# microsoft/UniSpeech

Hardware: AMD Instinct MI355X
Metric: audio-seconds/sec pretraining, WavLM-Base 15s@16kHz (higher is better)
Workload: dtype bf16; 1 GPU; WavLM-Base (12L, d=768) pretrain fwd+bwd+grad-reduce+fused-Adam, bf16, batch=32x15s per GPU, masked-pred loss (BASELINE.json configs[1]); global_batch=32, frames_per_utt=749, parallelism=dp1, optimizer=fused Adam, fp32 master, clip 10

## Files before the change

include/wavlm_hip.h:

```cpp
#ifndef WAVLM_HIP_H
#define WAVLM_HIP_H
#include <stddef.h>
#include <stdint.h>
#ifdef __cplusplus
extern "C" {
#endif

#define WAVLM_HIP_ABI_VERSION 29
int wavlm_abi_version(void);

typedef struct wavlm_gemm_desc {
  int32_t dtype;
  int32_t c_dtype;
  int32_t M, N, K, KB;
  int32_t transA, transB;
  int64_t lda, ldb, ldc;
  int64_t sA_kb, sB_kb;
  int32_t batch_o, batch_i;
  int64_t sA_o, sA_i, sB_o, sB_i, sC_o, sC_i;
  const void* A;
  const void* B;
  void* C;
  float alpha;
  int32_t epi;
  const void* bias; int32_t bias_dtype; int64_t sBias_o, sBias_i;
  void* aux; int32_t aux_dtype; int64_t ld_aux, sAux_o, sAux_i;
  const void* res; int32_t res_dtype; int64_t ld_res, sRes_o, sRes_i;
  int32_t accumulate;
  int32_t split_k;
  void* workspace; uint64_t ws_bytes;
  void* colsum; int32_t colsum_dtype; int32_t colsum_accumulate;
} wavlm_gemm_desc;

uint64_t wavlm_gemm_workspace_bytes(const wavlm_gemm_desc* d);
int wavlm_gemm(const wavlm_gemm_desc* d, void* stream);
int wavlm_gemm_grouped(const wavlm_gemm_desc* d, int32_t n, void* stream);

int32_t wavlm_grid_blocks(void);
int32_t wavlm_split_single(int32_t M, int32_t N, int64_t ktiles, int32_t grid);
int32_t wavlm_split_grouped(int64_t tiles, int64_t ktiles, int32_t grid, int32_t forced);
int32_t wavlm_slabs_grouped(int64_t tiles, int64_t ktiles, int32_t grid, int32_t forced, int32_t balanced);
// ... 3 lines not shown
  const void* dy;
  const void* x;
  void* dW;
  int32_t N, K;
} wavlm_wgrad_item;
uint64_t wavlm_linear_wgrads_workspace_bytes(const wavlm_wgrad_item* items, int32_t n_items, int64_t rows);
int wavlm_linear_wgrads(const wavlm_wgrad_item* items, int32_t n_items, int64_t rows, int32_t c_dtype, void* workspace,
                        uint64_t ws_bytes, void* stream);


int wavlm_layernorm_fwd(const void* x, const void* r, void* y, void* s, float* mean, float* rstd, const void* gamma,
                        const void* beta, int64_t rows, int32_t D, float eps, int32_t dtype, int32_t param_dtype,
                        int32_t act, float p_in, uint64_t seed_in, float p_out, uint64_t seed_out, void* stream);
uint64_t wavlm_layernorm_bwd_workspace_bytes(int32_t D);
int wavlm_layernorm_bwd(const void* dy, const void* s, const float* mean, const float* rstd, const void* gamma,
                        const void* beta, void* dx, void* dr, const void* dx_add, void* dgamma, void* dbeta,
                        void* dr_colsum, int64_t rows, int32_t D, int32_t dtype, int32_t param_dtype, int32_t act,
                        float p_in, uint64_t seed_in, float p_out, uint64_t seed_out, float grad_scale,
                        int32_t accumulate_params, int32_t dr_incl_add, void* workspace, uint64_t ws_bytes, void* stream);
int wavlm_layernorm_bwd_seg(const void* dy, const void* s, const float* mean, const float* rstd, const void* gamma,
                            const void* beta, void* dx, void* dr, const void* dx_add, void* dgamma, void* dbeta,
                            void* dr_colsum, int64_t rows, int32_t D, int32_t dtype, int32_t param_dtype, int32_t act,
                            float p_in, uint64_t seed_in, float p_out, uint64_t seed_out, float grad_scale,
                            int32_t accumulate_params, int32_t dr_incl_add, int32_t dx_seg_rows, int32_t dx_seg_gap,
                            void* workspace, uint64_t ws_bytes, void* stream);

uint64_t wavlm_colsum_workspace_bytes(int32_t N);
int wavlm_colsum(const void* x, int64_t rows, int32_t N, int64_t ld, int32_t dtype, const uint8_t* include_mask,
                 const uint8_t* exclude_mask, void* out, int32_t out_dtype, int32_t accumulate, void* workspace,
                 uint64_t ws_bytes, void* stream);

int wavlm_select_rows(const void* x, void* y, const uint8_t* sel, const void* emb, const uint8_t* zero, int64_t rows,
                      int32_t D, int32_t dtype, int32_t emb_dtype, void* stream);
int wavlm_gather_rows(const void* src, const int32_t* idx, void* dst, int64_t n_out, int32_t D, int32_t dtype,
                      void* stream);
#define WL_CONV_RELAYOUT_MAX 8
typedef struct {
  const void* W[WL_CONV_RELAYOUT_MAX];
  void* Wf[WL_CONV_RELAYOUT_MAX];
  void* Wb[WL_CONV_RELAYOUT_MAX];
  int32_t Cout[WL_CONV_RELAYOUT_MAX], Cin[WL_CONV_RELAYOUT_MAX], k[WL_CONV_RELAYOUT_MAX], s[WL_CONV_RELAYOUT_MAX];
  int32_t n_layers, dtype;
} wavlm_conv_relayout_desc;
int wavlm_conv_weights_relayout(const wavlm_conv_relayout_desc* d, void* stream);
int wavlm_conv_wgrad_scatter(const wavlm_conv_relayout_desc* d, int32_t accumulate, void* stream);
int wavlm_axpby(const void* x, int32_t x_dtype, void* y, int32_t y_dtype, int64_t n, float a, float b, void* stream);
int wavlm_scale_dev(void* y, int32_t dtype, int64_t n, const float* scalar, float extra, void* stream);
int wavlm_dropout(const void* x, void* y, int64_t n, float p, uint64_t seed, int32_t dtype, void* stream);
int wavlm_dropout_add(const void* x, const void* r, void* y, int64_t n, float p, uint64_t seed, int32_t dtype, void* stream);
uint64_t wavlm_sumsq_workspace_bytes(void);
int wavlm_sumsq(const void* x, int32_t dtype, int64_t n, float scale, float* out, void* workspace, uint64_t ws_bytes,
                void* stream);

uint64_t wavlm_conv0_gn_workspace_bytes(int32_t B, int64_t T, int32_t C, int32_t stride);
int wavlm_conv0_gn_gelu_fwd(const void* wav, int32_t wav_dtype, const void* W, const void* gamma, const void* beta,
                            int32_t param_dtype, void* out, int32_t out_dtype, float* stats, int32_t B, int64_t T,
                            int32_t C, int32_t kw, int32_t stride, float eps, void* workspace, uint64_t ws_bytes,
                            void* stream);
uint64_t wavlm_conv0_gn_bwd_workspace_bytes(int32_t B, int64_t T, int32_t C, int32_t stride);
int wavlm_conv0_gn_gelu_bwd(const void* wav, int32_t wav_dtype, const void* W, const void* gamma, const void* beta,
                            int32_t param_dtype, const void* g, int32_t g_dtype, const float* stats, void* dW,
                            void* dgamma, void* dbeta, int32_t B, int64_t T, int32_t C, int32_t kw, int32_t stride,
                            float gscale, void* workspace, uint64_t ws_bytes, void* stream);

uint64_t wavlm_conv0_ln_fwd_workspace_bytes(void);
int wavlm_conv0_ln_gelu_fwd(const void* wav, int32_t wav_dtype, const void* W, const void* conv_bias, const void* gamma,
// ... 224 lines not shown
```

unispeech_amd/_lib.py:

```python
import ctypes as C
import os

_HERE = os.path.dirname(os.path.abspath(__file__))
LIB_PATH = os.environ.get("WAVLM_HIP_LIB") or os.path.join(_HERE, "lib", "libwavlm_hip.so")

_lib = None
ABI_VERSION = 29

F32, BF16, I16 = 0, 1, 2

c_i32, c_i64, c_u64, c_f32, c_vp = C.c_int32, C.c_int64, C.c_uint64, C.c_float, C.c_void_p


class ConvRelayoutDesc(C.Structure):
    _fields_ = [("W", c_vp * 8), ("Wf", c_vp * 8), ("Wb", c_vp * 8),
                ("Cout", c_i32 * 8), ("Cin", c_i32 * 8), ("k", c_i32 * 8), ("s", c_i32 * 8),
                ("n_layers", c_i32), ("dtype", c_i32)]


class GemmDesc(C.Structure):
    _fields_ = [
        ("dtype", c_i32), ("c_dtype", c_i32),
        ("M", c_i32), ("N", c_i32), ("K", c_i32), ("KB", c_i32),
        ("transA", c_i32), ("transB", c_i32),
        ("lda", c_i64), ("ldb", c_i64), ("ldc", c_i64),
        ("sA_kb", c_i64), ("sB_kb", c_i64),
        ("batch_o", c_i32), ("batch_i", c_i32),
        ("sA_o", c_i64), ("sA_i", c_i64), ("sB_o", c_i64), ("sB_i", c_i64), ("sC_o", c_i64), ("sC_i", c_i64),
        ("A", c_vp), ("B", c_vp), ("C", c_vp),
        ("alpha", c_f32), ("epi", c_i32),
        ("bias", c_vp), ("bias_dtype", c_i32), ("sBias_o", c_i64), ("sBias_i", c_i64),
        ("aux", c_vp), ("aux_dtype", c_i32), ("ld_aux", c_i64), ("sAux_o", c_i64), ("sAux_i", c_i64),
        ("res", c_vp), ("res_dtype", c_i32), ("ld_res", c_i64), ("sRes_o", c_i64), ("sRes_i", c_i64),
        ("accumulate", c_i32), ("split_k", c_i32),
        ("workspace", c_vp), ("ws_bytes", c_u64),
        ("colsum", c_vp), ("colsum_dtype", c_i32), ("colsum_accumulate", c_i32),
    ]


class WgradItem(C.Structure):
# ... 17 lines not shown
        ("tab", c_vp), ("kpm", c_vp),
        ("x", c_vp), ("r_in", c_vp), ("y", c_vp), ("r_out", c_vp),
        ("saved", c_vp), ("saved_bytes", c_u64), ("workspace", c_vp), ("ws_bytes", c_u64),
        ("dy", c_vp), ("dr_out", c_vp), ("dx", c_vp), ("dr_in", c_vp), ("dtab", c_vp),
    ]


GRAD_LISTENER = C.CFUNCTYPE(None, c_vp, c_u64, c_vp, c_vp)


SIGNATURES = {
    "wavlm_abi_version": (c_i32, []),
    "wavlm_gemm_workspace_bytes": (c_u64, [C.POINTER(GemmDesc)]),
    "wavlm_gemm": (c_i32, [C.POINTER(GemmDesc), c_vp]),
    "wavlm_gemm_grouped": (c_i32, [C.POINTER(GemmDesc), c_i32, c_vp]),
    "wavlm_grid_blocks": (c_i32, []),
    "wavlm_split_single": (c_i32, [c_i32, c_i32, c_i64, c_i32]),
    "wavlm_split_grouped": (c_i32, [c_i64, c_i64, c_i32, c_i32]),
    "wavlm_slabs_grouped": (c_i32, [c_i64, c_i64, c_i32, c_i32, c_i32]),
    "wavlm_wgrad_grouping": (c_i32, []),
    "wavlm_linear_wgrads_workspace_bytes": (c_u64, [C.POINTER(WgradItem), c_i32, c_i64]),
    "wavlm_linear_wgrads": (c_i32, [C.POINTER(WgradItem), c_i32, c_i64, c_i32, c_vp, c_u64, c_vp]),
    "wavlm_layernorm_fwd": (c_i32, [c_vp, c_vp, c_vp, c_vp, c_vp, c_vp, c_vp, c_vp, c_i64, c_i32, c_f32, c_i32, c_i32,
                                    c_i32, c_f32, c_u64, c_f32, c_u64, c_vp]),
    "wavlm_layernorm_bwd_workspace_bytes": (c_u64, [c_i32]),
    "wavlm_layernorm_bwd": (c_i32, [c_vp, c_vp, c_vp, c_vp, c_vp, c_vp, c_vp, c_vp, c_vp, c_vp, c_vp, c_vp, c_i64, c_i32, c_i32,
                                    c_i32, c_i32, c_f32, c_u64, c_f32, c_u64, c_f32, c_i32, c_i32, c_vp, c_u64, c_vp]),
    "wavlm_layernorm_bwd_seg": (c_i32, [c_vp, c_vp, c_vp, c_vp, c_vp, c_vp, c_vp, c_vp, c_vp, c_vp, c_vp, c_vp, c_i64, c_i32, c_i32,
                                        c_i32, c_i32, c_f32, c_u64, c_f32, c_u64, c_f32, c_i32, c_i32, c_i32, c_i32, c_vp, c_u64,
                                        c_vp]),
    "wavlm_colsum_workspace_bytes": (c_u64, [c_i32]),
    "wavlm_colsum": (c_i32, [c_vp, c_i64, c_i32, c_i64, c_i32, c_vp, c_vp, c_vp, c_i32, c_i32, c_vp, c_u64, c_vp]),
    "wavlm_select_rows": (c_i32, [c_vp, c_vp, c_vp, c_vp, c_vp, c_i64, c_i32, c_i32, c_i32, c_vp]),
    "wavlm_gather_rows": (c_i32, [c_vp, c_vp, c_vp, c_i64, c_i32, c_i32, c_vp]),
    "wavlm_conv_weights_relayout": (c_i32, [C.POINTER(ConvRelayoutDesc), c_vp]),
    "wavlm_conv_wgrad_scatter": (c_i32, [C.POINTER(ConvRelayoutDesc), c_i32, c_vp]),
    "wavlm_axpby": (c_i32, [c_vp, c_i32, c_vp, c_i32, c_i64, c_f32, c_f32, c_vp]),
    "wavlm_scale_dev": (c_i32, [c_vp, c_i32, c_i64, c_vp, c_f32, c_vp]),
    "wavlm_dropout": (c_i32, [c_vp, c_vp, c_i64, c_f32, c_u64, c_i32, c_vp]),
    "wavlm_dropout_add": (c_i32, [c_vp, c_vp, c_vp, c_i64, c_f32, c_u64, c_i32, c_vp]),
    "wavlm_sumsq_workspace_bytes": (c_u64, []),
    "wavlm_sumsq": (c_i32, [c_vp, c_i32, c_i64, c_f32, c_vp, c_vp, c_u64, c_vp]),
    "wavlm_conv0_gn_workspace_bytes": (c_u64, [c_i32, c_i64, c_i32, c_i32]),
    "wavlm_conv0_gn_gelu_fwd": (c_i32, [c_vp, c_i32, c_vp, c_vp, c_vp, c_i32, c_vp, c_i32, c_vp, c_i32, c_i64, c_i32,
                                        c_i32, c_i32, c_f32, c_vp, c_u64, c_vp]),
    "wavlm_conv0_gn_bwd_workspace_bytes": (c_u64, [c_i32, c_i64, c_i32, c_i32]),
    "wavlm_conv0_gn_gelu_bwd": (c_i32, [c_vp, c_i32, c_vp, c_vp, c_vp, c_i32, c_vp, c_i32, c_vp, c_vp, c_vp, c_vp,
                                        c_i32, c_i64, c_i32, c_i32, c_i32, c_f32, c_vp, c_u64, c_vp]),
    "wavlm_conv0_ln_fwd_workspace_bytes": (c_u64, []),
    "wavlm_conv0_ln_gelu_fwd": (c_i32, [c_vp, c_i32, c_vp, c_vp, c_vp, c_vp, c_i32, c_vp, c_i32, c_i32, c_i64, c_i32, c_i32,
                                        c_i32, c_f32, c_vp, c_u64, c_vp]),
    "wavlm_conv0_ln_bwd_workspace_bytes": (c_u64, [c_i32, c_i64, c_i32, c_i32]),
    "wavlm_conv0_ln_gelu_bwd": (c_i32, [c_vp, c_i32, c_vp, c_vp, c_vp, c_vp, c_i32, c_vp, c_i32, c_vp, c_vp, c_vp, c_vp, c_i32,
                                        c_i64, c_i32, c_i32, c_i32, c_f32, c_f32, c_vp, c_u64, c_vp]),
    "wavlm_relpos_gather": (c_i32, [c_vp, c_i32, c_vp, c_vp, c_i32, c_i32, c_vp]),
    "wavlm_relpos_scatter": (c_i32, [c_vp, c_vp, c_vp, c_i32, c_i32, c_i32, c_i32, c_vp]),
    "wavlm_gate_fwd": (c_i32, [c_vp, c_vp, c_vp, c_vp, c_vp, c_vp, c_vp, c_i32, c_i32, c_i32, c_i32, c_i32, c_i32,
                               c_vp]),
    "wavlm_gate_bwd_workspace_bytes": (c_u64, [c_i32, c_i32]),
    "wavlm_gate_bwd": (c_i32, [c_vp, c_vp, c_vp, c_vp, c_vp, c_vp, c_vp, c_vp, c_vp, c_vp, c_i32, c_i32, c_i32, c_i32,
                               c_i32, c_i32, c_i32, c_vp, c_u64, c_vp]),
    "wavlm_attn_softmax_fwd": (c_i32, [c_vp, c_vp, c_vp, c_vp, c_vp, c_vp, c_i32, c_i32, c_i32, c_i64, c_i64, c_i32,
                                       c_i32, c_f32, c_u64, c_vp]),
    "wavlm_attn_softmax_bwd_workspace_bytes": (c_u64, [c_i32, c_i32, c_i32]),
    "wavlm_attn_softmax_bwd": (c_i32, [c_vp, c_vp, c_vp, c_vp, c_vp, c_vp, c_vp, c_vp, c_vp, c_i32, c_i32, c_i32,
                                       c_i32, c_i64, c_i64, c_i32, c_i32, c_f32, c_u64, c_vp, c_u64, c_vp]),
# ... 127 lines not shown
```

unispeech_amd/csrc/rowops.hip:

```cpp
#include "common.hpp"
#include <stdlib.h>
#include "../../include/wavlm_hip.h"

__device__ __forceinline__ void load8(const float* p, float (&v)[8]) {
  const float4 a = *reinterpret_cast<const float4*>(p);
  const float4 b = *reinterpret_cast<const float4*>(p + 4);
  v[0] = a.x; v[1] = a.y; v[2] = a.z; v[3] = a.w; v[4] = b.x; v[5] = b.y; v[6] = b.z; v[7] = b.w;
}
__device__ __forceinline__ void load8(const bf16_t* p, float (&v)[8]) {
  const uint4 a = *reinterpret_cast<const uint4*>(p);
  v[0] = __uint_as_float(a.x << 16); v[1] = __uint_as_float(a.x & 0xffff0000u);
  v[2] = __uint_as_float(a.y << 16); v[3] = __uint_as_float(a.y & 0xffff0000u);
  v[4] = __uint_as_float(a.z << 16); v[5] = __uint_as_float(a.z & 0xffff0000u);
  v[6] = __uint_as_float(a.w << 16); v[7] = __uint_as_float(a.w & 0xffff0000u);
}
__device__ __forceinline__ void store8(float* p, const float (&v)[8]) {
  *reinterpret_cast<float4*>(p) = make_float4(v[0], v[1], v[2], v[3]);
  *reinterpret_cast<float4*>(p + 4) = make_float4(v[4], v[5], v[6], v[7]);
}
__device__ __forceinline__ void store8(bf16_t* p, const float (&v)[8]) {
  uint4 o;
  o.x = pack_bf16x2(v[0], v[1]); o.y = pack_bf16x2(v[2], v[3]);
  o.z = pack_bf16x2(v[4], v[5]); o.w = pack_bf16x2(v[6], v[7]);
  *reinterpret_cast<uint4*>(p) = o;
// ... 610 lines not shown
#pragma unroll
    for (int e = 0; e < 8; ++e) acc[c][e] = 0.f;
  for (long row = (long)blockIdx.x * 4 + wave; row < rows; row += (long)gridDim.x * 4) {
    if (inc && !inc[row]) continue;
    if (exc && exc[row]) continue;
#pragma unroll
    for (int c = 0; c < CS_MAXC; ++c) {
      const int ch = lane + 64 * c;
      if (ch < nch) {
        float v[8];
        load8(x + row * ld + ch * 8, v);
#pragma unroll
        for (int e = 0; e < 8; ++e) acc[c][e] += v[e];
      }
    }
  }
  float* pg = part + (long)blockIdx.x * N;
#pragma unroll
  for (int c = 0; c < CS_MAXC; ++c) {
    __syncthreads();
#pragma unroll
    for (int e = 0; e < 8; ++e) red[wave][lane * 8 + e] = acc[c][e];
    __syncthreads();
    for (int i = threadIdx.x; i < 512; i += 256) {
      const int ch = (i >> 3) + 64 * c;
      if (ch < nch) pg[ch * 8 + (i & 7)] = red[0][i] + red[1][i] + red[2][i] + red[3][i];
    }
  }
}

template <typename T, typename TP>
__global__ __launch_bounds__(256) void select_rows_kernel(const T* __restrict__ x, T* __restrict__ y,
    const unsigned char* __restrict__ sel, const TP* __restrict__ emb, const unsigned char* __restrict__ zero,
    long rows, int D) {
  const int nch = D >> 3;
  const long total = rows * nch;
  for (long i = (long)blockIdx.x * blockDim.x + threadIdx.x; i < total; i += (long)gridDim.x * blockDim.x) {
    const long row = i / nch; const int ch = (int)(i - row * nch);
    float v[8];
    if (zero && zero[row]) {
#pragma unroll
      for (int e = 0; e < 8; ++e) v[e] = 0.f;
    } else if (sel && sel[row]) {
      if (emb) load8(emb + ch * 8, v);
      else {
#pragma unroll
        for (int e = 0; e < 8; ++e) v[e] = 0.f;
      }
    } else {
      load8(x + row * D + ch * 8, v);
    }
    store8(y + row * D + ch * 8, v);
  }
}

template <typename T>
__global__ __launch_bounds__(256) void gather_rows_kernel(const T* __restrict__ src, const int* __restrict__ idx,
                                                           T* __restrict__ dst, long n_out, int D) {
  const int nch = D >> 3;
  const long total = n_out * nch;
  for (long i = (long)blockIdx.x * blockDim.x + threadIdx.x; i < total; i += (long)gridDim.x * blockDim.x) {
    const long row = i / nch; const int ch = (int)(i - row * nch);
    const int srow = idx[row];
    float v[8];
    if (srow >= 0) load8(src + (long)srow * D + ch * 8, v);
    else {
#pragma unroll
      for (int e = 0; e < 8; ++e) v[e] = 0.f;
    }
    store8(dst + row * D + ch * 8, v);
  }
}

__global__ __launch_bounds__(256) void axpby_kernel(const void* x, int xdt, void* y, int ydt, long n, float a, float b) {
  for (long i = (long)blockIdx.x * blockDim.x + threadIdx.x; i < n; i += (long)gridDim.x * blockDim.x) {
    float v = a * ld_elem(x, i, xdt);
    if (b != 0.f) v += b * ld_elem(y, i, ydt);
    st_elem(y, i, ydt, v);
  }
}


__global__ __launch_bounds__(256) void scale_dev_kernel(void* y, int ydt, long n, const float* __restrict__ s, float extra) {
// ... 288 lines not shown
  WL_LAUNCH(colsum_finish_kernel, dim3((unsigned)((n + 15) / 16)), dim3(1024), 0, st, part, nblk, (long)n, n, out, out_dtype,
            accumulate, 0L, (void*)nullptr, (void*)nullptr);
  return wl_check_launch();
}
extern "C" {

uint64_t wavlm_colsum_workspace_bytes(int32_t N) { return (uint64_t)CS_BLOCKS * N * sizeof(float); }

int wavlm_colsum(const void* x, int64_t rows, int32_t N, int64_t ld, int32_t dtype, const uint8_t* include_mask,
                 const uint8_t* exclude_mask, void* out, int32_t out_dtype, int32_t accumulate, void* workspace,
                 uint64_t ws_bytes, void* stream) {
  if (!x || !out || !workspace || rows < 0 || N <= 0 || (N & 7) || N > CS_MAXC * 512 || (ld & 7)) return WL_EINVAL;
  if (ws_bytes < wavlm_colsum_workspace_bytes(N)) return WL_EINVAL;
  hipStream_t st = (hipStream_t)stream;
  const unsigned grid = grid_for(rows > 0 ? rows : 1, 4, CS_BLOCKS);
  float* part = (float*)workspace;
  if (dtype == WL_F32)
    WL_LAUNCH((colsum_partial_kernel<float>), dim3(grid), dim3(256), 0, st, (const float*)x, (long)rows, (int)N,
                       (long)ld, include_mask, exclude_mask, part);
  else if (dtype == WL_BF16)
    WL_LAUNCH((colsum_partial_kernel<bf16_t>), dim3(grid), dim3(256), 0, st, (const bf16_t*)x, (long)rows, (int)N,
                       (long)ld, include_mask, exclude_mask, part);
  else return WL_EINVAL;
  int rc = wl_check_launch();
  if (rc != WL_OK) return rc;
  if (wl_fin_add(part, (int)grid, (long)N, N, out, out_dtype, accumulate)) return WL_OK;
  WL_LAUNCH(colsum_finish_kernel, dim3((unsigned)((N + 15) / 16)), dim3(1024), 0, st, part, (int)grid, (long)N,
                     (int)N, out, (int)out_dtype, (int)accumulate, 0L, (void*)nullptr, (void*)nullptr);
  rc = wl_check_launch();
  if (rc == WL_OK && accumulate) wl_notify_grad(out, (uint64_t)N * wl_esize(out_dtype), stream);
  return rc;
}

int wavlm_select_rows(const void* x, void* y, const uint8_t* sel, const void* emb, const uint8_t* zero, int64_t rows,
                      int32_t D, int32_t dtype, int32_t emb_dtype, void* stream) {
  if (!x || !y || rows < 0 || D <= 0 || (D & 7)) return WL_EINVAL;
  if (rows == 0) return WL_OK;
  hipStream_t st = (hipStream_t)stream;
  const unsigned grid = grid_for(rows * (D >> 3), 256, 4096);
#define SEL(T, TP) WL_LAUNCH((select_rows_kernel<T, TP>), dim3(grid), dim3(256), 0, st, (const T*)x, (T*)y, sel, \
    (const TP*)emb, zero, (long)rows, (int)D)
  if (dtype == WL_F32 && emb_dtype == WL_F32) SEL(float, float);
  else if (dtype == WL_BF16 && emb_dtype == WL_BF16) SEL(bf16_t, bf16_t);
  else if (dtype == WL_BF16 && emb_dtype == WL_F32) SEL(bf16_t, float);
  else return WL_EINVAL;
#undef SEL
  return wl_check_launch();
}

int wavlm_gather_rows(const void* src, const int32_t* idx, void* dst, int64_t n_out, int32_t D, int32_t dtype,
                      void* stream) {
  if (!src || !idx || !dst || n_out < 0 || D <= 0 || (D & 7)) return WL_EINVAL;
  if (n_out == 0) return WL_OK;
  hipStream_t st = (hipStream_t)stream;
  const unsigned grid = grid_for(n_out * (D >> 3), 256, 4096);
  if (dtype == WL_F32)
    WL_LAUNCH((gather_rows_kernel<float>), dim3(grid), dim3(256), 0, st, (const float*)src, idx, (float*)dst,
                       (long)n_out, (int)D);
  else if (dtype == WL_BF16)
    WL_LAUNCH((gather_rows_kernel<bf16_t>), dim3(grid), dim3(256), 0, st, (const bf16_t*)src, idx, (bf16_t*)dst,
                       (long)n_out, (int)D);
  else return WL_EINVAL;
  return wl_check_launch();
}

int wavlm_conv_weights_relayout(const wavlm_conv_relayout_desc* d, void* stream) {
  if (!d || d->n_layers < 1 || d->n_layers > WL_CONV_RELAYOUT_MAX || (d->dtype != WL_F32 && d->dtype != WL_BF16)) return WL_EINVAL;
  long mx = 0;
  for (int l = 0; l < d->n_layers; ++l) {
    if (!d->W[l] || !d->Wf[l] || d->Cout[l] <= 0 || d->Cin[l] <= 0 || d->k[l] <= 0 || d->s[l] <= 0 || d->s[l] > d->k[l]) return WL_EINVAL;
    const long n = (long)d->Cout[l] * d->Cin[l] * d->k[l];
    if (n > mx) mx = n;
  }
  const unsigned gx = grid_for(mx, 256, 8192);
  WL_LAUNCH(conv_weights_relayout_kernel, dim3(gx, (unsigned)d->n_layers), dim3(256), 0, (hipStream_t)stream, *d);
  return wl_check_launch();
}

int wavlm_conv_wgrad_scatter(const wavlm_conv_relayout_desc* d, int32_t accumulate, void* stream) {
  if (!d || d->n_layers < 1 || d->n_layers > WL_CONV_RELAYOUT_MAX || (d->dtype != WL_F32 && d->dtype != WL_BF16)) return WL_EINVAL;
// ... 82 lines not shown
```

unispeech_amd/functional.py:

```python
import os
import threading
import weakref

import torch

from . import ops

_SEED_CTR = [0]
USE_FUSED_ATTENTION = True
_ASP = os.environ.get("WAVLM_ATTN_STORE_P", "0")
ATTN_STORE_P = True if _ASP == "1" else ("bits" if _ASP in ("bits", "2") else False)


def next_seed():
    _SEED_CTR[0] += 1
    return (torch.initial_seed() * 0x9E3779B97F4A7C15 + _SEED_CTR[0] * 0xD1B54A32D192ED03) & 0xFFFFFFFFFFFFFFFF


def _rup(x, m):
    return (x + m - 1) // m * m


CHAIN_CONSUMERS = os.environ.get("WAVLM_CHAIN_CONSUMERS", "1") == "1"
WGRAD_GROUPING = None
SINK_LISTENERS = []


def h2d(a, dev):
    t = torch.from_numpy(a) if not torch.is_tensor(a) else a
    dev = torch.device(dev)
    if dev.type != "cuda" or t.device.type != "cpu" or t.numel() == 0:
        return t.to(dev)
    return t.pin_memory().to(dev, non_blocking=True)


_SINK_USES = {}


def reset_sink_uses():
    _SINK_USES.clear()
    _PADDED_GRAD[0] = None


def _sink_use(p, explicit=None):
    if not SINK_LISTENERS:
        return
    t = explicit if explicit is not None else _sink(p)
    if t is not None:
        k = t.data_ptr()
        _SINK_USES[k] = _SINK_USES.get(k, 0) + 1


def _sink_written(t):
    if not SINK_LISTENERS:
        return
    k = t.data_ptr()
    left = _SINK_USES.get(k, 1) - 1
    if left > 0:
        _SINK_USES[k] = left
        return
    _SINK_USES.pop(k, None)
    for cb in SINK_LISTENERS:
        cb(t)


def _sink(p):
# ... 716 lines not shown
            dqkv, dgate, dtab = ops.attn_fused_bwd(qkvc, O, dO.contiguous(), lse, gate, tab, kpm, H, scale, p_drop, seed,
                                                   dbias=sb.view(-1) if sb is not None else None, dbias_accumulate=True,
                                                   pstore=pstore)
            if sb is not None:
                _sink_written(sb)
            return dqkv, dgate, dtab, None, None, None, None, None, None, None
        qkvc, S, P, lse, gate, tab, kpm = ctx.saved_tensors
        B, T, D, H, hd, ld, scale, p_drop, seed = ctx.cfg
        D3 = 3 * D
        dev = dO.device
        dOc = dO.contiguous()
        dP = torch.empty((B * H, T, ld), dtype=P.dtype, device=dev)
        ops.gemm(dOc, qkvc, dP, T, T, hd, lda=D, ldb=D3, ldc=ld, batch=(B, H), sA=(T * D, hd), sB=(T * D3, hd),
                 b_off=2 * D, sC=(H * T * ld, T * ld))
        dS = torch.empty_like(dP)
        dgate = dtab = None
        if tab is not None:
            dgate = torch.empty((B, H, T), dtype=torch.float32, device=dev)
            dtab = torch.empty_like(tab)
        ops.attn_softmax_bwd(S, dP, lse, gate, tab, kpm, dS, dgate, dtab, B, H, T, ld, ld, p_drop, seed)
        dqkv = torch.empty_like(qkvc)
        ops.gemm(dS, qkvc, dqkv, T, hd, T, lda=ld, ldb=D3, ldc=D3, transB=True, batch=(B, H),
                 sA=(H * T * ld, T * ld), sB=(T * D3, hd), b_off=D, sC=(T * D3, hd), c_off=0, alpha=scale)
        ops.gemm(dS, qkvc, dqkv, T, hd, T, lda=ld, ldb=D3, ldc=D3, transA=True, transB=True, batch=(B, H),
                 sA=(H * T * ld, T * ld), sB=(T * D3, hd), b_off=0, sC=(T * D3, hd), c_off=D, alpha=scale)
        ops.gemm(P, dOc, dqkv, T, hd, T, lda=ld, ldb=D, ldc=D3, transA=True, transB=True, batch=(B, H),
                 sA=(H * T * ld, T * ld), sB=(T * D, hd), sC=(T * D3, hd), c_off=2 * D)
        return dqkv, dgate, dtab, None, None, None, None, None, None, None


class SelectRowsFn(torch.autograd.Function):

    @staticmethod
    def forward(ctx, x, sel, emb, zero):
        xc = x.contiguous()
        y = ops.select_rows(xc, sel, emb, zero)
        ctx.save_for_backward(sel, zero, emb)
        return y

    @staticmethod
    def backward(ctx, dy):
        sel, zero, emb = ctx.saved_tensors
        dyc = dy.contiguous()
        dx = ops.select_rows(dyc, sel, None, zero) if ctx.needs_input_grad[0] else None
        demb = None
        if emb is not None and sel is not None and ctx.needs_input_grad[2]:
            demb = ops.colsum(dyc.view(-1, dyc.shape[-1]), emb.dtype, include=sel, exclude=zero)
        return dx, None, demb, None


class GatherRowsFn(torch.autograd.Function):

    @staticmethod
    def forward(ctx, x2d, idx, inv_idx):
        ctx.save_for_backward(inv_idx)
        ctx.n = x2d.shape[0]
        if idx.numel() == 0:
            return x2d.new_empty((0, x2d.shape[1]))
        return ops.gather_rows(x2d.contiguous(), idx, idx.numel())

    @staticmethod
    def backward(ctx, dy):
        (inv_idx,) = ctx.saved_tensors
        if dy.shape[0] == 0:
            return dy.new_zeros((ctx.n, dy.shape[1])), None, None
        return ops.gather_rows(dy.contiguous(), inv_idx, ctx.n), None, None


class DropoutFn(torch.autograd.Function):
    @staticmethod
    def forward(ctx, x, p, seed):
        ctx.p, ctx.seed = p, seed
        return ops.dropout(x.contiguous(), p, seed)

    @staticmethod
    def backward(ctx, dy):
        return ops.dropout(dy.contiguous(), ctx.p, ctx.seed), None, None


def dropout(x, p, training=True):
    if not training or p <= 0:
# ... 245 lines not shown
```

unispeech_amd/ops.py:

```python
import ctypes as C
import os

import torch

from . import _lib
from ._lib import BF16, F32, ConvRelayoutDesc, GemmDesc, check

_WS = {}


def dt(t):
    if t.dtype == torch.float32:
        return F32
    if t.dtype == torch.bfloat16:
        return BF16
    raise TypeError("unsupported dtype %s (float32 / bfloat16 only)" % t.dtype)


def _dev(t):
    if not t.is_cuda:
        raise _lib.WavlmHipError("unispeech_amd kernels need a HIP device tensor (no CPU fallback)")
    return t.device


# ... 191 lines not shown
        if torch.is_tensor(dr_colsum):
            raise ValueError("dr_colsum sink needs dgamma / dbeta sinks")
        dr_colsum = torch.empty_like(gamma) if not acc else torch.zeros_like(gamma)
    L = _lib.lib()
    need = L.wavlm_layernorm_bwd_workspace_bytes(D)
    ws = workspace(dev, need)
    check(L.wavlm_layernorm_bwd_seg(ptr(dy), ptr(s), ptr(mean), ptr(rstd), ptr(gamma), ptr(beta), ptr(dx), ptr(dr),
                                    ptr(dx_add), ptr(dgamma), ptr(dbeta), ptr(dr_colsum), rows, D, dt(dy), dt(gamma), int(act),
                                    float(p_in), int(seed_in), float(p_out), int(seed_out), float(grad_scale), int(acc),
                                    int(bool(dr_incl_add)), seg_rows, seg_gap, ptr(ws), need, stream()), "wavlm_layernorm_bwd_seg")
    if padded is not None:
        dx._padded = padded
    return dx, dr, dgamma, dbeta, dr_colsum


def colsum(x2d, out_dtype, *, include=None, exclude=None, rows=None, N=None, ld=None, out=None, accumulate=False):
    dev = _dev(x2d)
    if rows is None:
        N = x2d.shape[-1]
        rows = x2d.numel() // N
        ld = N
        _contig(x2d)
    if out is None:
        out = torch.empty(N, dtype=out_dtype, device=dev)
        accumulate = False
    L = _lib.lib()
    need = L.wavlm_colsum_workspace_bytes(N)
    ws = workspace(dev, need)
    check(L.wavlm_colsum(ptr(x2d), rows, N, ld, dt(x2d), ptr(include), ptr(exclude), ptr(out), dt(out),
                         int(bool(accumulate)), ptr(ws), need, stream()), "wavlm_colsum")
    return out


def select_rows(x, sel, emb, zero):
    _dev(x); _contig(x)
    D = x.shape[-1]
    rows = x.numel() // D
    y = torch.empty_like(x)
    check(_lib.lib().wavlm_select_rows(ptr(x), ptr(y), ptr(sel), ptr(emb), ptr(zero), rows, D, dt(x),
                                       dt(emb) if emb is not None else dt(x), stream()), "wavlm_select_rows")
    return y


def gather_rows(src2d, idx, n_out):
    dev = _dev(src2d); _contig(src2d)
    D = src2d.shape[-1]
    dst = torch.empty((n_out, D), dtype=src2d.dtype, device=dev)
    check(_lib.lib().wavlm_gather_rows(ptr(src2d), ptr(idx), ptr(dst), n_out, D, dt(src2d), stream()),
          "wavlm_gather_rows")
    return dst


def _conv_desc(weights, specs):
    d = ConvRelayoutDesc()
    if len(weights) > 8:
        raise ValueError("at most 8 convolution layers per call")
    d.n_layers, d.dtype = len(weights), dt(weights[0])
    for l, (W, (k, s_)) in enumerate(zip(weights, specs)):
        _dev(W); _contig(W)
        Cout, Cin, kk = W.shape
        if kk != k:
            raise ValueError("kernel width of layer %d does not match its spec" % l)
        d.Cout[l], d.Cin[l], d.k[l], d.s[l] = Cout, Cin, k, s_
        d.W[l] = W.data_ptr()
    return d


def conv_weights_relayout(weights, specs, want_bwd):
    d = _conv_desc(weights, specs)
    Wf, Wb = [], []
    for l, (W, (k, s_)) in enumerate(zip(weights, specs)):
        Cout, Cin, _ = W.shape
        f = torch.empty((Cout, k * Cin), dtype=W.dtype, device=W.device)
# ... 544 lines not shown
```

unispeech_amd/pretrain.py:

```python
import math
from dataclasses import dataclass, field
from typing import Dict, List, Optional, Tuple

import numpy as np
import torch
import torch.nn as nn

from . import functional as F
from .wavlm import ConvFeatureExtractionModel, TransformerEncoder, WavLM


@dataclass
class WavLMPretrainConfig:
    label_rate: int = 50
    extractor_mode: str = "default"
    encoder_layers: int = 12
    encoder_embed_dim: int = 768
    encoder_ffn_embed_dim: int = 3072
    encoder_attention_heads: int = 12
    activation_fn: str = "gelu"
    dropout: float = 0.1
    attention_dropout: float = 0.1
    activation_dropout: float = 0.0
    encoder_layerdrop: float = 0.0
# ... 147 lines not shown
        import os
        force = os.environ.get("WAVLM_VALIDATE_TARGETS") == "1"
        for i, t in enumerate(target_list):
            if t.numel() == 0 or not (force or t.device.type == "cpu"):
                continue
            V = self.num_classes[min(i, len(self.num_classes) - 1)]
            lo, hi = (int(v) for v in torch.aminmax(t))
            if lo < 0 or hi >= V:
                raise IndexError("label set %d holds ids in [%d, %d] but its dictionary has %d entries" % (i, lo, hi, V))

    def _mask_numpy(self, B, T, padding_cpu, boundary):
        if self.mask_prob <= 0:
            return None
        if boundary is not None and len(boundary) == B:
            from .masking import compute_mask_indices
            m = np.full((B, T), False)
            for i in range(B):
                if len(boundary[i]) > 0:
                    start, end = boundary[i][:-1], boundary[i][1:]
                    coin = np.random.binomial(1, 0.5, size=len(start))
                    for j in np.argwhere(coin == 1)[:, 0]:
                        m[i][start[j]:end[j]] = True
                else:
                    m[i] = compute_mask_indices((1, T), None, self.mask_prob, self.mask_length, self.mask_selection,
                                                self.mask_other, min_masks=2, no_overlap=self.no_mask_overlap,
                                                min_space=self.mask_min_space)
            return m
        return self.compute_mask(B, T, padding_cpu)

    def forward(self, source: torch.Tensor, target_list: Optional[List[torch.Tensor]] = None,
                padding_mask: Optional[torch.Tensor] = None, boundary=None, mask: bool = True,
                features_only: bool = False, output_layer: Optional[int] = None,
                padding_mask_cpu: Optional[torch.Tensor] = None) -> Dict[str, torch.Tensor]:
        x, feats = self._features(source)
        B, T, _ = x.shape
        dev = x.device
        target_inds = None
        if target_list is not None:
            new_T, target_inds = self.forward_targets(T, target_list)
            if new_T != T:
                x = x[:, :new_T].contiguous()
                feats = feats[:, :new_T].contiguous()
                T = new_T
        features_pen = F.FeaturesPenFn.apply(feats, self.feat_grad_scale) if not features_only else None

        pad_cpu = None
        if padding_mask is not None:
            if padding_mask_cpu is not None:
                pad_cpu = self.forward_padding_mask(T, padding_mask_cpu)
                padding_mask = F.h2d(pad_cpu, dev)
            else:
                padding_mask = self.forward_padding_mask(T, padding_mask)
                pad_cpu = padding_mask.cpu()
        x = F.dropout(x, self.dropout_input.p, self.training)

        mask_np = None
        if mask:
            mask_np = self._mask_numpy(B, T, pad_cpu, boundary if self.boundary_mask else None)
        sel = F.h2d(mask_np.astype(np.uint8), dev).view(-1) if mask_np is not None else None
        enc_pad = padding_mask
        if padding_mask is not None and pad_cpu is not None and not bool(pad_cpu.any()):
            enc_pad = None
        kpm = enc_pad.to(torch.uint8).contiguous().view(-1) if enc_pad is not None else None
        if sel is not None or kpm is not None:
            x = F.SelectRowsFn.apply(x, sel, self.mask_emb if sel is not None else None, kpm)
        if mask:
            x = self.apply_channel_mask(x)
        layer = None if output_layer is None else output_layer - 1
        if self.predict_layers is not None and not features_only:
            layer = list(self.predict_layers)
        spk_x = None
        if self.utterance_contrastive_layer is not None:
            x, layer_results, conv_sum, spk_x = self.encoder(x, padding_mask=enc_pad, layer=layer,
                                                             fairseq_layer_results=True, prezeroed=True,
                                                             extract_layer=self.utterance_contrastive_layer - 1)
        else:
            x, layer_results, conv_sum = self.encoder(x, padding_mask=enc_pad, layer=layer,
                                                      fairseq_layer_results=True, prezeroed=True)
        result = {"x": x, "padding_mask": padding_mask, "features": conv_sum, "layer_results": layer_results}
        if features_only:
            if output_layer is not None and getattr(self, "post_layer_norm", None) is not None:
                ln = self.post_layer_norm[-1]
                result["x"] = F.layer_norm(x, ln.weight, ln.bias, ln.eps)[0]
            return result
        self._check_targets(target_list)

        pad_np = pad_cpu.numpy() if pad_cpu is not None else np.zeros((B, T), dtype=bool)
        m_np = mask_np if mask_np is not None else np.zeros((B, T), dtype=bool)
        def layer_head(li):
            fp = self.final_proj[li] if self.separate_label_embeds else self.final_proj
            lec = self.label_embs_concat
            if lec.dim() == 3:
                lec = lec[li] if (self.separate_label_embeds or self.separate_layer_targets) else lec[0]
            if self.separate_layer_targets:
                return fp, [(lec[:self.num_classes[li]], target_list[li])], False
            return fp, list(zip(lec.split(self.num_classes, 0), target_list)), self.untie_final_proj

        n = B * T
        if self.predict_layers is not None:
            taps = [lx.transpose(0, 1) for lx, _ in layer_results]
            if hasattr(self, "post_layer_norm") and self.post_layer_norm is not None:
                taps = [F.layer_norm(t, ln.weight, ln.bias, ln.eps)[0] for t, ln in zip(taps, self.post_layer_norm)]
            sources = [t.reshape(B * T, -1) for t in taps]
        else:
            sources = [x.reshape(B * T, -1)]

        tinds_np = target_inds.numpy().astype(np.int64)

        def head(frame_sel_np, need_grad):
            out = []
            for li, x2d in enumerate(sources):
                out.extend(head_one(x2d, frame_sel_np, need_grad, li))
            return out

        def head_one(x2d, frame_sel_np, need_grad, li=0):
            with torch.set_grad_enabled(bool(need_grad) and torch.is_grad_enabled()):
                return head_body(x2d, frame_sel_np, need_grad, li)

        def head_body(x2d, frame_sel_np, need_grad, li):
            idx_np = np.flatnonzero(frame_sel_np.reshape(-1)).astype(np.int32)
            S = int(idx_np.size)
            inv_np = np.full(n, -1, dtype=np.int32)
            inv_np[idx_np] = np.arange(S, dtype=np.int32)
            idx = F.h2d(idx_np, dev)
            inv = F.h2d(inv_np, dev)
            rows = F.GatherRowsFn.apply(x2d, idx, inv)
            fp, pairs, untied = layer_head(li)
            proj = F.LinearFn.apply(rows, fp.weight, fp.bias)
            projs = proj.chunk(len(pairs), dim=-1) if untied else [proj] * len(pairs)
            out = []
            bsel, fsel = np.divmod(idx_np.astype(np.int64), T)
            flat_cache = {}
            for pj, (emb, t) in zip(projs, pairs):
                if self.target_glu is not None:
                    tg = self.target_glu[0]
                    emb = F.GLUFn.apply(F.LinearFn.apply(emb.contiguous(), tg.weight, tg.bias))
                Tl = int(t.size(1))
                if Tl not in flat_cache:
                    flat_cache[Tl] = F.h2d(bsel * Tl + tinds_np[fsel], t.device)
                tt = t.contiguous().view(-1).index_select(0, flat_cache[Tl]).to(torch.int32)
                loss, ncorrect = F.MaskedPredLossFn.apply(pj.contiguous(), emb, tt, self.logit_temp, need_grad)
                out.append({"loss": loss, "correct": ncorrect, "count": S, "proj": pj, "target": tt, "label_embs": emb})
            return out

        result["masked"] = head(np.logical_and(~pad_np, m_np), True) if not self.skip_masked else None
        result["nomask"] = head(np.logical_and(~pad_np, ~m_np), self.training_nomask_grad) \
            if not self.skip_nomask else None
        result["logit_m_list"] = None
        result["logit_u_list"] = None
        result["features_pen"] = features_pen
        if self.utterance_contrastive_loss:
            if self.skip_masked or spk_x is None:
                result.update(loss_spk_m=None, mean_targets=None, contrastive_acc=None, loss_spk_u=None)
            else:
                loss_spk, mean_t, acc, q = self._utterance_contrastive(spk_x, np.logical_and(~pad_np, m_np))
                result.update(loss_spk_m=loss_spk, mean_targets=mean_t, contrastive_acc=acc, loss_spk_u=None)
                if q is not None:
                    result.update(prob_perplexity=q["prob_perplexity"], code_perplexity=q["code_perplexity"],
                                  num_vars=q["num_vars"], temp=q["temp"])
        return result

    instance_sampling = "host"

    def _sample_instances(self, bsz, tsz, num, device=None):
        n_in, n_cr = self.n_instances, self.cross_sample_instances
        high, cross_high = tsz, tsz * bsz
        assert high > 1
        idxs = cross = None
        if n_in > 0:
            tszs = torch.arange(num, device=device).unsqueeze(-1).expand(-1, n_in).flatten()
            idxs = torch.randint(low=0, high=high - 1, size=(bsz, n_in * num), device=device)
            idxs[idxs >= tszs] += 1
        if n_cr > 0:
            tszs = torch.arange(num, device=device).unsqueeze(-1).expand(-1, n_cr).flatten()
            cross = torch.randint(low=0, high=cross_high - 1, size=(bsz, n_cr * num), device=device)
            cross[cross >= tszs] += 1
        if n_in > 0:
            for i in range(1, bsz):
                idxs[i] += i * high
        else:
            idxs = cross
        if n_cr > 0 and n_in > 0:
            idxs = torch.cat([idxs, cross], dim=1)
        return idxs

    def _utterance_contrastive(self, spk_x, masked_np):
        B, T, D = spk_x.shape
        dev = spk_x.device
        idx_np = np.flatnonzero(masked_np.reshape(-1)).astype(np.int32)
        S = int(idx_np.size)
        num = S // B
        assert num * B == S and num > 1
        inv_np = np.full(B * T, -1, dtype=np.int32)
        inv_np[idx_np] = np.arange(S, dtype=np.int32)
        rows = F.GatherRowsFn.apply(spk_x.reshape(B * T, D), F.h2d(idx_np, dev), F.h2d(inv_np, dev))
# ... 208 lines not shown
```

Before: 15460 audio-s/s.

## Pack host-side index uploads into one H2D and fuse input dropout into select_rows

```diff
diff --git a/include/wavlm_hip.h b/include/wavlm_hip.h
--- a/include/wavlm_hip.h
+++ b/include/wavlm_hip.h
@@ -6,7 +6,7 @@
 extern "C" {
 #endif
 
-#define WAVLM_HIP_ABI_VERSION 29
+#define WAVLM_HIP_ABI_VERSION 30
 int wavlm_abi_version(void);
 
 typedef struct wavlm_gemm_desc {
@@ -76,6 +76,8 @@
 
 int wavlm_select_rows(const void* x, void* y, const uint8_t* sel, const void* emb, const uint8_t* zero, int64_t rows,
                       int32_t D, int32_t dtype, int32_t emb_dtype, void* stream);
+int wavlm_select_rows_dropout(const void* x, void* y, const uint8_t* sel, const void* emb, const uint8_t* zero, int64_t rows,
+                              int32_t D, int32_t dtype, int32_t emb_dtype, float p, uint64_t seed, void* stream);
 int wavlm_gather_rows(const void* src, const int32_t* idx, void* dst, int64_t n_out, int32_t D, int32_t dtype,
                       void* stream);
 #define WL_CONV_RELAYOUT_MAX 8
diff --git a/unispeech_amd/_lib.py b/unispeech_amd/_lib.py
--- a/unispeech_amd/_lib.py
+++ b/unispeech_amd/_lib.py
@@ -5,7 +5,7 @@
 LIB_PATH = os.environ.get("WAVLM_HIP_LIB") or os.path.join(_HERE, "lib", "libwavlm_hip.so")
 
 _lib = None
-ABI_VERSION = 29
+ABI_VERSION = 30
 
 F32, BF16, I16 = 0, 1, 2
 
@@ -89,6 +89,7 @@
     "wavlm_colsum_workspace_bytes": (c_u64, [c_i32]),
     "wavlm_colsum": (c_i32, [c_vp, c_i64, c_i32, c_i64, c_i32, c_vp, c_vp, c_vp, c_i32, c_i32, c_vp, c_u64, c_vp]),
     "wavlm_select_rows": (c_i32, [c_vp, c_vp, c_vp, c_vp, c_vp, c_i64, c_i32, c_i32, c_i32, c_vp]),
+    "wavlm_select_rows_dropout": (c_i32, [c_vp, c_vp, c_vp, c_vp, c_vp, c_i64, c_i32, c_i32, c_i32, c_f32, c_u64, c_vp]),
     "wavlm_gather_rows": (c_i32, [c_vp, c_vp, c_vp, c_i64, c_i32, c_i32, c_vp]),
     "wavlm_conv_weights_relayout": (c_i32, [C.POINTER(ConvRelayoutDesc), c_vp]),
     "wavlm_conv_wgrad_scatter": (c_i32, [C.POINTER(ConvRelayoutDesc), c_i32, c_vp]),
diff --git a/unispeech_amd/csrc/rowops.hip b/unispeech_amd/csrc/rowops.hip
--- a/unispeech_amd/csrc/rowops.hip
+++ b/unispeech_amd/csrc/rowops.hip
@@ -666,7 +666,7 @@
 template <typename T, typename TP>
 __global__ __launch_bounds__(256) void select_rows_kernel(const T* __restrict__ x, T* __restrict__ y,
     const unsigned char* __restrict__ sel, const TP* __restrict__ emb, const unsigned char* __restrict__ zero,
-    long rows, int D) {
+    long rows, int D, unsigned th, float sc, unsigned long long seed) {
   const int nch = D >> 3;
   const long total = rows * nch;
   for (long i = (long)blockIdx.x * blockDim.x + threadIdx.x; i < total; i += (long)gridDim.x * blockDim.x) {
@@ -683,6 +683,11 @@
       }
     } else {
       load8(x + row * D + ch * 8, v);
+      if (th) {
+        const unsigned k = keep8(seed, (unsigned long long)i * 8, th);
+#pragma unroll
+        for (int e = 0; e < 8; ++e) v[e] = ((k >> e) & 1u) ? v[e] * sc : 0.f;
+      }
     }
     store8(y + row * D + ch * 8, v);
   }
@@ -1037,20 +1042,27 @@
   return rc;
 }
 
-int wavlm_select_rows(const void* x, void* y, const uint8_t* sel, const void* emb, const uint8_t* zero, int64_t rows,
-                      int32_t D, int32_t dtype, int32_t emb_dtype, void* stream) {
-  if (!x || !y || rows < 0 || D <= 0 || (D & 7)) return WL_EINVAL;
+int wavlm_select_rows_dropout(const void* x, void* y, const uint8_t* sel, const void* emb, const uint8_t* zero, int64_t rows,
+                              int32_t D, int32_t dtype, int32_t emb_dtype, float p, uint64_t seed, void* stream) {
+  if (!x || !y || rows < 0 || D <= 0 || (D & 7) || p < 0.f || p >= 1.f) return WL_EINVAL;
   if (rows == 0) return WL_OK;
   hipStream_t st = (hipStream_t)stream;
+  const unsigned th = drop_thresh(p);
+  const float sc = 1.f / (1.f - p);
   const unsigned grid = grid_for(rows * (D >> 3), 256, 4096);
 #define SEL(T, TP) WL_LAUNCH((select_rows_kernel<T, TP>), dim3(grid), dim3(256), 0, st, (const T*)x, (T*)y, sel, \
-    (const TP*)emb, zero, (long)rows, (int)D)
+    (const TP*)emb, zero, (long)rows, (int)D, th, sc, (unsigned long long)seed)
   if (dtype == WL_F32 && emb_dtype == WL_F32) SEL(float, float);
   else if (dtype == WL_BF16 && emb_dtype == WL_BF16) SEL(bf16_t, bf16_t);
   else if (dtype == WL_BF16 && emb_dtype == WL_F32) SEL(bf16_t, float);
   else return WL_EINVAL;
 #undef SEL
   return wl_check_launch();
+}
+
+int wavlm_select_rows(const void* x, void* y, const uint8_t* sel, const void* emb, const uint8_t* zero, int64_t rows,
+                      int32_t D, int32_t dtype, int32_t emb_dtype, void* stream) {
+  return wavlm_select_rows_dropout(x, y, sel, emb, zero, rows, D, dtype, emb_dtype, 0.f, 0, stream);
 }
 
 int wavlm_gather_rows(const void* src, const int32_t* idx, void* dst, int64_t n_out, int32_t D, int32_t dtype,
diff --git a/unispeech_amd/functional.py b/unispeech_amd/functional.py
--- a/unispeech_amd/functional.py
+++ b/unispeech_amd/functional.py
@@ -2,6 +2,7 @@
 import threading
 import weakref
 
+import numpy as np
 import torch
 
 from . import ops
@@ -32,6 +33,42 @@
     if dev.type != "cuda" or t.device.type != "cpu" or t.numel() == 0:
         return t.to(dev)
     return t.pin_memory().to(dev, non_blocking=True)
+
+
+_UPLOAD_RING = {}
+
+
+def h2d_packed(arrays, dev):
+    dev = torch.device(dev)
+    keys = list(arrays)
+    offs, total = [], 0
+    for k in keys:
+        offs.append(total)
+        total += _rup(arrays[k].nbytes, 256)
+    if dev.type != "cuda" or total == 0:
+        return {k: h2d(arrays[k], dev) for k in keys}
+    ring = _UPLOAD_RING.setdefault(dev.index if dev.index is not None else torch.cuda.current_device(), [0, [[None, None], [None, None]]])
+    slot = ring[1][ring[0]]
+    ring[0] ^= 1
+    if slot[1] is not None:
+        slot[1].synchronize()
+    if slot[0] is None or slot[0].numel() < total:
+        slot[0] = torch.empty(max(total, 1 << 16), dtype=torch.uint8, pin_memory=True)
+    stage = slot[0].numpy()
+    for k, o in zip(keys, offs):
+        a = np.ascontiguousarray(arrays[k])
+        stage[o:o + a.nbytes] = a.reshape(-1).view(np.uint8)
+    with torch.cuda.device(dev):
+        buf = slot[0][:total].to(dev, non_blocking=True)
+        if slot[1] is None:
+            slot[1] = torch.cuda.Event()
+        slot[1].record()
+    out = {}
+    for k, o in zip(keys, offs):
+        a = arrays[k]
+        tdt = torch.from_numpy(np.empty(0, dtype=a.dtype)).dtype
+        out[k] = buf[o:o + a.nbytes].view(tdt).view(a.shape)
+    return out
 
 
 _SINK_USES = {}
@@ -814,21 +851,22 @@
 class SelectRowsFn(torch.autograd.Function):
 
     @staticmethod
-    def forward(ctx, x, sel, emb, zero):
+    def forward(ctx, x, sel, emb, zero, p=0.0, seed=0):
         xc = x.contiguous()
-        y = ops.select_rows(xc, sel, emb, zero)
+        y = ops.select_rows(xc, sel, emb, zero, p, seed)
         ctx.save_for_backward(sel, zero, emb)
+        ctx.p, ctx.seed = p, seed
         return y
 
     @staticmethod
     def backward(ctx, dy):
         sel, zero, emb = ctx.saved_tensors
         dyc = dy.contiguous()
-        dx = ops.select_rows(dyc, sel, None, zero) if ctx.needs_input_grad[0] else None
+        dx = ops.select_rows(dyc, sel, None, zero, ctx.p, ctx.seed) if ctx.needs_input_grad[0] else None
         demb = None
         if emb is not None and sel is not None and ctx.needs_input_grad[2]:
             demb = ops.colsum(dyc.view(-1, dyc.shape[-1]), emb.dtype, include=sel, exclude=zero)
-        return dx, None, demb, None
+        return dx, None, demb, None, None, None
 
 
 class GatherRowsFn(torch.autograd.Function):
diff --git a/unispeech_amd/ops.py b/unispeech_amd/ops.py
--- a/unispeech_amd/ops.py
+++ b/unispeech_amd/ops.py
@@ -247,13 +247,18 @@
     return out
 
 
-def select_rows(x, sel, emb, zero):
+def select_rows(x, sel, emb, zero, p=0.0, seed=0):
     _dev(x); _contig(x)
     D = x.shape[-1]
     rows = x.numel() // D
     y = torch.empty_like(x)
-    check(_lib.lib().wavlm_select_rows(ptr(x), ptr(y), ptr(sel), ptr(emb), ptr(zero), rows, D, dt(x),
-                                       dt(emb) if emb is not None else dt(x), stream()), "wavlm_select_rows")
+    edt = dt(emb) if emb is not None else dt(x)
+    if p > 0:
+        check(_lib.lib().wavlm_select_rows_dropout(ptr(x), ptr(y), ptr(sel), ptr(emb), ptr(zero), rows, D, dt(x), edt,
+                                                   float(p), int(seed), stream()), "wavlm_select_rows_dropout")
+    else:
+        check(_lib.lib().wavlm_select_rows(ptr(x), ptr(y), ptr(sel), ptr(emb), ptr(zero), rows, D, dt(x), edt, stream()),
+              "wavlm_select_rows")
     return y
 
 
diff --git a/unispeech_amd/pretrain.py b/unispeech_amd/pretrain.py
--- a/unispeech_amd/pretrain.py
+++ b/unispeech_amd/pretrain.py
@@ -203,38 +203,91 @@
                 padding_mask: Optional[torch.Tensor] = None, boundary=None, mask: bool = True,
                 features_only: bool = False, output_layer: Optional[int] = None,
                 padding_mask_cpu: Optional[torch.Tensor] = None) -> Dict[str, torch.Tensor]:
+        dev = source.device
+        B = source.shape[0]
+        packed = (self.packed_upload and dev.type == "cuda" and source.dim() == 2
+                  and (padding_mask is None or padding_mask_cpu is not None))
+        host, ondev = {}, {}
+
+        def devt(key):
+            if key not in ondev:
+                ondev[key] = F.h2d(host[key], dev)
+            return ondev[key]
+
+        def host_side(T):
+            target_inds = None
+            if target_list is not None:
+                T, target_inds = self.forward_targets(T, target_list)
+            pad_cpu = None
+            if padding_mask is not None and padding_mask_cpu is not None:
+                pad_cpu = self.forward_padding_mask(T, padding_mask_cpu)
+                host["pad"] = pad_cpu.numpy()
+            return T, target_inds, pad_cpu
+
+        def draw_mask(T, pad_cpu):
+            mask_np = self._mask_numpy(B, T, pad_cpu, boundary if self.boundary_mask else None) if mask else None
+            if mask_np is not None:
+                host["sel"] = mask_np.astype(np.uint8)
+            return mask_np
+
+        def head_arrays(T, target_inds, pad_cpu, mask_np):
+            pad_np = pad_cpu.numpy() if pad_cpu is not None else np.zeros((B, T), dtype=bool)
+            m_np = mask_np if mask_np is not None else np.zeros((B, T), dtype=bool)
+            tinds_np = target_inds.numpy().astype(np.int64)
+            widths = sorted({int(t.size(1)) for t in target_list})
+            for tag, skip, fs in (("m", self.skip_masked, np.logical_and(~pad_np, m_np)),
+                                  ("u", self.skip_nomask, np.logical_and(~pad_np, ~m_np))):
+                if skip:
+                    continue
+                idx_np = np.flatnonzero(fs.reshape(-1)).astype(np.int32)
+                inv_np = np.full(B * T, -1, dtype=np.int32)
+                inv_np[idx_np] = np.arange(idx_np.size, dtype=np.int32)
+                host[tag, "idx"], host[tag, "inv"] = idx_np, inv_np
+                bsel, fsel = np.divmod(idx_np.astype(np.int64), T)
+                for Tl in widths:
+                    host[tag, "flat", Tl] = bsel * Tl + tinds_np[fsel]
+
+        want_heads = target_list is not None and not features_only
+        if packed:
+            T = source.shape[1]
+            for k, s in self.feature_extractor.specs:
+                T = (T - k) // s + 1
+            T_new, target_inds, pad_cpu = host_side(T)
+            mask_np = draw_mask(T_new, pad_cpu)
+            if want_heads:
+                head_arrays(T_new, target_inds, pad_cpu, mask_np)
+            ondev.update(F.h2d_packed(host, dev))
         x, feats = self._features(source)
-        B, T, _ = x.shape
-        dev = x.device
-        target_inds = None
-        if target_list is not None:
-            new_T, target_inds = self.forward_targets(T, target_list)
-            if new_T != T:
-                x = x[:, :new_T].contiguous()
-                feats = feats[:, :new_T].contiguous()
-                T = new_T
+        if packed and x.shape[1] != T:
+            raise RuntimeError("the extractor gave %d frames where its layer specs give %d" % (x.shape[1], T))
+        T = x.shape[1]
+        if not packed:
+            T_new, target_inds, pad_cpu = host_side(T)
+        if T_new != T:
+            x = x[:, :T_new].contiguous()
+            feats = feats[:, :T_new].contiguous()
+            T = T_new
         features_pen = F.FeaturesPenFn.apply(feats, self.feat_grad_scale) if not features_only else None
 
-        pad_cpu = None
         if padding_mask is not None:
-            if padding_mask_cpu is not None:
-                pad_cpu = self.forward_padding_mask(T, padding_mask_cpu)
-                padding_mask = F.h2d(pad_cpu, dev)
+            if pad_cpu is not None:
+                padding_mask = devt("pad")
             else:
                 padding_mask = self.forward_padding_mask(T, padding_mask)
                 pad_cpu = padding_mask.cpu()
-        x = F.dropout(x, self.dropout_input.p, self.training)
-
-        mask_np = None
-        if mask:
-            mask_np = self._mask_numpy(B, T, pad_cpu, boundary if self.boundary_mask else None)
-        sel = F.h2d(mask_np.astype(np.uint8), dev).view(-1) if mask_np is not None else None
+        if not packed:
+            mask_np = draw_mask(T, pad_cpu)
+        sel = devt("sel").view(-1) if mask_np is not None else None
         enc_pad = padding_mask
         if padding_mask is not None and pad_cpu is not None and not bool(pad_cpu.any()):
             enc_pad = None
         kpm = enc_pad.to(torch.uint8).contiguous().view(-1) if enc_pad is not None else None
+        p_in = self.dropout_input.p if self.training else 0.0
         if sel is not None or kpm is not None:
-            x = F.SelectRowsFn.apply(x, sel, self.mask_emb if sel is not None else None, kpm)
+            x = F.SelectRowsFn.apply(x, sel, self.mask_emb if sel is not None else None, kpm, p_in,
+                                     F.next_seed() if p_in > 0 else 0)
+        else:
+            x = F.dropout(x, p_in, self.training)
         if mask:
             x = self.apply_channel_mask(x)
         layer = None if output_layer is None else output_layer - 1
@@ -256,8 +309,9 @@
             return result
         self._check_targets(target_list)
 
-        pad_np = pad_cpu.numpy() if pad_cpu is not None else np.zeros((B, T), dtype=bool)
-        m_np = mask_np if mask_np is not None else np.zeros((B, T), dtype=bool)
+        if not packed:
+            head_arrays(T, target_inds, pad_cpu, mask_np)
+
         def layer_head(li):
             fp = self.final_proj[li] if self.separate_label_embeds else self.final_proj
             lec = self.label_embs_concat
@@ -267,7 +321,6 @@
                 return fp, [(lec[:self.num_classes[li]], target_list[li])], False
             return fp, list(zip(lec.split(self.num_classes, 0), target_list)), self.untie_final_proj
 
-        n = B * T
         if self.predict_layers is not None:
             taps = [lx.transpose(0, 1) for lx, _ in layer_results]
             if hasattr(self, "post_layer_norm") and self.post_layer_norm is not None:
@@ -276,47 +329,36 @@
         else:
             sources = [x.reshape(B * T, -1)]
 
-        tinds_np = target_inds.numpy().astype(np.int64)
-
-        def head(frame_sel_np, need_grad):
+        def head(tag, need_grad):
             out = []
             for li, x2d in enumerate(sources):
-                out.extend(head_one(x2d, frame_sel_np, need_grad, li))
+                out.extend(head_one(x2d, tag, need_grad, li))
             return out
 
-        def head_one(x2d, frame_sel_np, need_grad, li=0):
+        def head_one(x2d, tag, need_grad, li=0):
             with torch.set_grad_enabled(bool(need_grad) and torch.is_grad_enabled()):
-                return head_body(x2d, frame_sel_np, need_grad, li)
-
-        def head_body(x2d, frame_sel_np, need_grad, li):
-            idx_np = np.flatnonzero(frame_sel_np.reshape(-1)).astype(np.int32)
-            S = int(idx_np.size)
-            inv_np = np.full(n, -1, dtype=np.int32)
-            inv_np[idx_np] = np.arange(S, dtype=np.int32)
-            idx = F.h2d(idx_np, dev)
-            inv = F.h2d(inv_np, dev)
-            rows = F.GatherRowsFn.apply(x2d, idx, inv)
+                return head_body(x2d, tag, need_grad, li)
+
+        def head_body(x2d, tag, need_grad, li):
+            S = int(host[tag, "idx"].size)
+            rows = F.GatherRowsFn.apply(x2d, devt((tag, "idx")), devt((tag, "inv")))
             fp, pairs, untied = layer_head(li)
             proj = F.LinearFn.apply(rows, fp.weight, fp.bias)
             projs = proj.chunk(len(pairs), dim=-1) if untied else [proj] * len(pairs)
             out = []
-            bsel, fsel = np.divmod(idx_np.astype(np.int64), T)
-            flat_cache = {}
             for pj, (emb, t) in zip(projs, pairs):
                 if self.target_glu is not None:
                     tg = self.target_glu[0]
                     emb = F.GLUFn.apply(F.LinearFn.apply(emb.contiguous(), tg.weight, tg.bias))
-                Tl = int(t.size(1))
-                if Tl not in flat_cache:
-                    flat_cache[Tl] = F.h2d(bsel * Tl + tinds_np[fsel], t.device)
-                tt = t.contiguous().view(-1).index_select(0, flat_cache[Tl]).to(torch.int32)
+                key = (tag, "flat", int(t.size(1)))
+                flat = devt(key) if t.device == dev else F.h2d(host[key], t.device)
+                tt = t.contiguous().view(-1).index_select(0, flat).to(torch.int32)
                 loss, ncorrect = F.MaskedPredLossFn.apply(pj.contiguous(), emb, tt, self.logit_temp, need_grad)
                 out.append({"loss": loss, "correct": ncorrect, "count": S, "proj": pj, "target": tt, "label_embs": emb})
             return out
 
-        result["masked"] = head(np.logical_and(~pad_np, m_np), True) if not self.skip_masked else None
-        result["nomask"] = head(np.logical_and(~pad_np, ~m_np), self.training_nomask_grad) \
-            if not self.skip_nomask else None
+        result["masked"] = head("m", True) if not self.skip_masked else None
+        result["nomask"] = head("u", self.training_nomask_grad) if not self.skip_nomask else None
         result["logit_m_list"] = None
         result["logit_u_list"] = None
         result["features_pen"] = features_pen
@@ -324,6 +366,8 @@
             if self.skip_masked or spk_x is None:
                 result.update(loss_spk_m=None, mean_targets=None, contrastive_acc=None, loss_spk_u=None)
             else:
+                pad_np = pad_cpu.numpy() if pad_cpu is not None else np.zeros((B, T), dtype=bool)
+                m_np = mask_np if mask_np is not None else np.zeros((B, T), dtype=bool)
                 loss_spk, mean_t, acc, q = self._utterance_contrastive(spk_x, np.logical_and(~pad_np, m_np))
                 result.update(loss_spk_m=loss_spk, mean_targets=mean_t, contrastive_acc=acc, loss_spk_u=None)
                 if q is not None:
@@ -332,6 +376,7 @@
         return result
 
     instance_sampling = "host"
+    packed_upload = True
 
     def _sample_instances(self, bsz, tsz, num, device=None):
         n_in, n_cr = self.n_instances, self.cross_sample_instances
```

Result: no change. 15560 audio-s/s, median of 6 (+0.6%).
